# oceanusxiv/pathtracer-rs

Measured on NVIDIA B200. Metric: samples/sec, higher is better.
Workload: dtype f32

## Files before the change

pathtracer_rs_b200/csrc/dev_accel.cuh:

```cuda
#pragma once
#include "dev_texture.cuh"

namespace ptrs {

struct RayPre {
  int kz;
  float sx, sy, sz;
};
PT_DEV V3 permute(V3 v, int kz) {
  const bool z0 = kz == 0, z1 = kz == 1;
  return mk3(z0 ? v.y : (z1 ? v.z : v.x), z0 ? v.z : (z1 ? v.x : v.y), z0 ? v.x : (z1 ? v.y : v.z));
}

PT_DEV RayPre ray_precompute(V3 d) {
  RayPre p;
  p.kz = max_dimension(vabs(d));
  const V3 dp = permute(d, p.kz);
  p.sx = -dp.x / dp.z;
  p.sy = -dp.y / dp.z;
  p.sz = 1.0f / dp.z;
  return p;
}

PT_DEV bool tri_core(V3 p0, V3 p1, V3 p2, V3 o, const RayPre& rp, float t_max, float* t_out, float* b0o, float* b1o, float* b2o) {
// ... 203 lines not shown

#ifndef PT_REFILL_IDLE
#define PT_REFILL_IDLE 8
#endif
#ifndef PT_SEARCH_MIN
#define PT_SEARCH_MIN 6
#endif

template <class Work>
PT_DEV void trace_empty(uint32_t n_items, uint32_t* ticket, Work& work) {
  DevHit miss;
  miss.prim = -1;
  miss.t = miss.b0 = miss.b1 = miss.b2 = 0.f;
  const int lane = threadIdx.x & 31;
  for (;;) {
    const uint32_t base = (lane == 0) ? atomicAdd(ticket, 32u) : 0u;
    const uint32_t b = __shfl_sync(0xffffffffu, base, 0);
    if (b >= n_items) return;
    const uint32_t i = b + lane;
    if (i < n_items) {
      LaneRay r;
      bool more = work.begin(i, &r);
      while (more) more = work.end(i, miss, false, &r);
    }
  }
}

#define PT_RB_NX 1u
#define PT_RB_NY 2u
#define PT_RB_NZ 4u
#define PT_RB_KZ_SHIFT 3
#define PT_RB_ANY 32u
#define PT_RB_LIVE 64u
#ifndef PT_BOX_STEPS
#define PT_BOX_STEPS 3
#endif
#ifndef PT_TRI_STEPS
#define PT_TRI_STEPS 1
#endif
#ifndef PT_EAGER_POP
#define PT_EAGER_POP 0
#endif
#ifndef PT_NEAR_LEAF_DIRECT
#define PT_NEAR_LEAF_DIRECT 0
#endif
#ifndef PT_SMEM_STACK
#define PT_SMEM_STACK 0
#endif
#ifndef PT_STACK8
#define PT_STACK8 0
#endif
#ifndef PT_PUSH_PREFETCH
#define PT_PUSH_PREFETCH 0
#endif
#ifndef PT_PARK_PREFETCH_ON
#define PT_PARK_PREFETCH_ON 0
#endif
#if PT_PARK_PREFETCH_ON
#define PT_PARK_PREFETCH(prim) asm volatile("prefetch.global.L1 [%0];" ::"l"(sc.tri_verts + 3 * (size_t)(prim)))
#else
#define PT_PARK_PREFETCH(prim) ((void)0)
#endif

#ifndef PT_TRACE_BLOCK
#define PT_TRACE_BLOCK 128
#endif
// ... 674 lines not shown
        RayPre rp;
        rp.kz = (int)((rbits >> PT_RB_KZ_SHIFT) & 3u);
        rp.sx = sx;
        rp.sy = sy;
        rp.sz = sz;
        float t, b0, b1, b2;
        if (tri_core(mk3(v0), mk3(v1), mk3(v2), o, rp, t_max, &t, &b0, &b1, &b2) &&
            !tri_post_reject(sc, (int)prim, mk3(v0), mk3(v1), mk3(v2), __float_as_uint(v2.w), b0, b1, b2, false)) {
          hit_prim = (int)prim;
          pl_cnt = 0;
          sp_ = 0;
          cur = PT_W_NONE;
        }
      }
    };
    for (;;) {
      const bool has = pl_cnt != 0u || PT_W_IS_LEAF(cur);
      if (__ballot_sync(FULL, has) == 0) break;
      tri_step();
    }

    if ((rbits & PT_RB_LIVE) && cur == PT_W_NONE && sp_ == 0 && pl_cnt == 0u) {
      DevHit h;
      h.prim = hit_prim;
      h.t = t_max;
      h.b0 = h.b1 = h.b2 = 0.f;
      LaneRay r;
      if (work.end(item, h, hit_prim >= 0, &r)) start_ray(r);
      else rbits = 0;
    }
  }
}

template <bool COUNT, bool DIST, class Work>
PT_DEV void trace_stream(const DevScene& sc, uint32_t n_items, uint32_t* ticket, Work& work, uint32_t* c_nodes, uint32_t* c_tris) {
  if (COUNT) trace_counted(sc, n_items, ticket, work, c_nodes, c_tris);
  else trace_fast<DIST>(sc, n_items, ticket, work);
}

}
```

pathtracer_rs_b200/csrc/k_trace.cu:

```cuda
#include "launch.hpp"
#include "wavefront.cuh"

#ifndef PT_TRACE_MIN_BLOCKS
#define PT_TRACE_MIN_BLOCKS 8
#endif

namespace ptrs {

PT_DEV uint32_t coalesced_slot(uint32_t* counter) {
  const uint32_t m = __activemask();
  const uint32_t grp = __match_any_sync(m, (unsigned long long)(uintptr_t)counter);
  const int lane = threadIdx.x & 31;
  const int leader = __ffs(grp) - 1;
  uint32_t base = 0;
  if (lane == leader) base = atomicAdd(counter, (uint32_t)__popc(grp));
  base = __shfl_sync(grp, base, leader);
  return base + (uint32_t)__popc(grp & ((1u << lane) - 1u));
}

struct ExtendWork {
  const DevScene& sc;
  const PathArrays& P;
  const int* __restrict__ q_ext;
  int* __restrict__ q_class;
  uint32_t cap;
  RoundCounters* ctr;
  int p;
  __device__ bool begin(uint32_t i, LaneRay* r) {
    p = q_ext[i];
    const PathRay pr = ld256(&P.slot[p].r);
    r->o = mk3(pr.ox, pr.oy, pr.oz);
    r->d = mk3(pr.dx, pr.dy, pr.dz);
    r->t_max = CUDART_INF_F;
    r->any_hit = false;
    return true;
  }
  __device__ bool end(uint32_t, const DevHit& h, bool found, LaneRay*) {
    const int cls = found ? sc.materials[__float_as_int(__ldg(&sc.tri_verts[3 * (size_t)h.prim].w))].type : PT_CLASS_MISS;
    const size_t slot = (size_t)cls * cap + coalesced_slot(&ctr->n_class[cls]);
    q_class[slot] = p;
    if (found) P.q_hit[slot] = make_float4(__int_as_float(h.prim), h.b0, h.b1, h.b2);
    return false;
  }
};

template <bool COUNT, bool DIST>
__global__ void __launch_bounds__(128, PT_TRACE_MIN_BLOCKS) extend_kernel(const __grid_constant__ DevScene sc, const __grid_constant__ PathArrays P, const int* __restrict__ q_ext, int* __restrict__ q_class,
                                                      uint32_t cap, RoundCounters* ctr, GlobalCounters* g) {
  uint32_t c_nodes = 0, c_tris = 0;
  ExtendWork w{sc, P, q_ext, q_class, cap, ctr, 0};
  trace_stream<COUNT, DIST>(sc, ctr->n_ext, &ctr->t_ext, w, &c_nodes, &c_tris);
  if (COUNT) {
    warp_sum_add(c_nodes, &g->nodes_tested);
    warp_sum_add(c_tris, &g->tris_tested);
  }
}

struct ConnectWork {
  const PathArrays& P;
  uint32_t n_low, top;
  uint32_t n_shadow, n_mis;
  uint32_t cur;
  __device__ bool begin(uint32_t i, LaneRay* r) {
    cur = P.q_ray[i < n_low ? i : top - (i - n_low)];
    const uint32_t rec = cur >> 1;
    if (cur & 1u) {
      const F8 n23 = ld256(reinterpret_cast<const F8*>(&P.nee[rec].n2));
      r->o = mk3(n23.a);
      r->d = mk3(n23.b);
      r->t_max = CUDART_INF_F;
      r->any_hit = (__float_as_uint(n23.b.w) & PT_NEE_MIS_ANY) != 0;
      ++n_mis;
    } else {
      const F8 n01 = ld256(reinterpret_cast<const F8*>(&P.nee[rec].n0));
      r->o = mk3(n01.a);
      r->d = mk3(n01.b);
      r->t_max = 1.0f - PT_SHADOW_EPSILON;
      r->any_hit = true;
      ++n_shadow;
    }
    return true;
  }
  __device__ bool end(uint32_t, const DevHit& h, bool found, LaneRay*) {
    NeeRes* res = P.nee_res + (cur >> 1);
    if (cur & 1u) *reinterpret_cast<float4*>(res) = make_float4(__int_as_float(found ? h.prim : -1), h.b0, h.b1, h.b2);
    else res->occluded = found ? 1u : 0u;
    return false;
  }
};

template <bool COUNT, bool DIST>
__global__ void __launch_bounds__(128, PT_TRACE_MIN_BLOCKS) connect_kernel(const __grid_constant__ DevScene sc, const __grid_constant__ PathArrays P, uint32_t cap,
                                                                           bool closest_only, RoundCounters* ctr, GlobalCounters* g) {
  uint32_t c_nodes = 0, c_tris = 0;
  const uint32_t n_low = closest_only ? 0u : ctr->n_ray;
  ConnectWork w{P, n_low, 2u * cap - 1u, 0u, 0u, 0u};
  trace_stream<COUNT, DIST>(sc, n_low + ctr->n_ray_closest, closest_only ? &ctr->t_ray_closest : &ctr->t_ray, w, &c_nodes, &c_tris);
  warp_sum_add(w.n_shadow, &g->shadow_rays);
  warp_sum_add(w.n_mis, &g->mis_rays);
  if (COUNT) {
    warp_sum_add(c_nodes, &g->nee_nodes_tested);
    warp_sum_add(c_tris, &g->nee_tris_tested);
  }
}

__global__ void __launch_bounds__(128, PT_TRACE_MIN_BLOCKS) occlusion_kernel(const __grid_constant__ DevScene sc, const __grid_constant__ PathArrays P, RoundCounters* ctr, GlobalCounters* g) {
  const uint32_t n = ctr->n_ray;
  ConnectWork w{P, n, 0u, 0u, 0u, 0u};
  trace_occlusion(sc, n, &ctr->t_ray, w);
  warp_sum_add(w.n_shadow, &g->shadow_rays);
  warp_sum_add(w.n_mis, &g->mis_rays);
}

struct IntersectWork {
  const PtrsRay* __restrict__ rays;
  PtrsHit* __restrict__ hits;
  uint8_t* __restrict__ occluded;
  bool any_hit;
  const uint32_t* __restrict__ prim_map;
  __device__ bool begin(uint32_t i, LaneRay* r) {
    const float* q = (const float*)(rays + i);
    r->o = mk3(__ldg(q), __ldg(q + 1), __ldg(q + 2));
    r->d = mk3(__ldg(q + 3), __ldg(q + 4), __ldg(q + 5));
    r->t_max = __ldg(q + 6);
    r->any_hit = any_hit;
    return true;
  }
  __device__ bool end(uint32_t i, const DevHit& h, bool found, LaneRay*) {
    if (any_hit) {
      occluded[i] = found ? 1 : 0;
    } else {
      PtrsHit out;
      out.prim = found ? (prim_map ? (int)__ldg(prim_map + h.prim) : h.prim) : -1;
      out.t = found ? h.t : 0.f;
      out.b0 = h.b0;
      out.b1 = h.b1;
      out.b2 = h.b2;
      hits[i] = out;
    }
    return false;
  }
};

template <bool ANY_HIT, bool COUNT, bool DIST>
__global__ void __launch_bounds__(128, PT_TRACE_MIN_BLOCKS) intersect_kernel(const __grid_constant__ DevScene sc, const PtrsRay* __restrict__ rays, uint32_t n, PtrsHit* __restrict__ hits,
                                                         uint8_t* __restrict__ occluded, uint32_t* ticket, GlobalCounters* g, const uint32_t* __restrict__ prim_map) {
  uint32_t c_nodes = 0, c_tris = 0;
  IntersectWork w{rays, hits, occluded, ANY_HIT, prim_map};
  trace_stream<COUNT, DIST>(sc, n, ticket, w, &c_nodes, &c_tris);
  if (COUNT) {
    warp_sum_add(c_nodes, &g->nodes_tested);
    warp_sum_add(c_tris, &g->tris_tested);
  }
}

__global__ void __launch_bounds__(128, PT_TRACE_MIN_BLOCKS) intersect_p_occlusion_kernel(const __grid_constant__ DevScene sc, const PtrsRay* __restrict__ rays, uint32_t n,
                                                                                         uint8_t* __restrict__ occluded, uint32_t* ticket) {
  IntersectWork w{rays, nullptr, occluded, true, nullptr};
  trace_occlusion(sc, n, ticket, w);
}

void launch_extend(cudaStream_t st, int sm, bool count, const DevScene& sc, const PathArrays& P, const int* q_ext, int* q_class, uint32_t cap,
                   RoundCounters* ctr, GlobalCounters* g) {
  if (count) extend_kernel<true, false><<<PT_GRID((extend_kernel<true, false>), 128, sm), 128, 0, st>>>(sc, P, q_ext, q_class, cap, ctr, g);
  else if (sc.dist_order) extend_kernel<false, true><<<PT_GRID((extend_kernel<false, true>), 128, sm), 128, 0, st>>>(sc, P, q_ext, q_class, cap, ctr, g);
  else extend_kernel<false, false><<<PT_GRID((extend_kernel<false, false>), 128, sm), 128, 0, st>>>(sc, P, q_ext, q_class, cap, ctr, g);
}
void launch_connect(cudaStream_t st, int sm, bool count, const DevScene& sc, const PathArrays& P, uint32_t cap, bool closest_only, RoundCounters* ctr,
                    GlobalCounters* g) {
  if (count) connect_kernel<true, false><<<PT_GRID((connect_kernel<true, false>), 128, sm), 128, 0, st>>>(sc, P, cap, closest_only, ctr, g);
  else if (sc.dist_order) connect_kernel<false, true><<<PT_GRID((connect_kernel<false, true>), 128, sm), 128, 0, st>>>(sc, P, cap, closest_only, ctr, g);
  else connect_kernel<false, false><<<PT_GRID((connect_kernel<false, false>), 128, sm), 128, 0, st>>>(sc, P, cap, closest_only, ctr, g);
}
void launch_occlusion(cudaStream_t st, int sm, const DevScene& sc, const PathArrays& P, RoundCounters* ctr, GlobalCounters* g) {
  occlusion_kernel<<<PT_GRID(occlusion_kernel, 128, sm), 128, 0, st>>>(sc, P, ctr, g);
}
void launch_intersect(cudaStream_t st, int sm, bool any_hit, bool count, const DevScene& sc, const PtrsRay* rays, uint32_t n, PtrsHit* hits,
                      uint8_t* occluded, uint32_t* ticket, GlobalCounters* g, const uint32_t* prim_map) {
#define PT_LAUNCH_INTERSECT(A, C, D) \
  intersect_kernel<A, C, D><<<PT_GRID((intersect_kernel<A, C, D>), 128, sm), 128, 0, st>>>(sc, rays, n, hits, occluded, ticket, g, prim_map)
  const bool dist = sc.dist_order != 0;
  if (any_hit && !count && sc.n_wnodes > 0) intersect_p_occlusion_kernel<<<PT_GRID(intersect_p_occlusion_kernel, 128, sm), 128, 0, st>>>(sc, rays, n, occluded, ticket);
  else if (!any_hit && count) PT_LAUNCH_INTERSECT(false, true, false);
  else if (any_hit && count) PT_LAUNCH_INTERSECT(true, true, false);
  else if (!any_hit && dist) PT_LAUNCH_INTERSECT(false, false, true);
  else if (!any_hit) PT_LAUNCH_INTERSECT(false, false, false);
  else if (dist) PT_LAUNCH_INTERSECT(true, false, true);
  else PT_LAUNCH_INTERSECT(true, false, false);
#undef PT_LAUNCH_INTERSECT
}

}
```

pathtracer_rs_b200/csrc/ptrs_b200.cu:

```cuda
#include <cuda_runtime.h>

#include <algorithm>
#include <cmath>
#include <cstdio>
#include <cstdlib>
#include <cstring>
#include <memory>
#include <mutex>
#include <string>
#include <vector>

#include "handles.hpp"
#include "launch.hpp"
#include "wavefront.cuh"

using namespace ptrs;

extern "C" const unsigned char ptrs_sobol_blob[];
extern "C" const unsigned char ptrs_sobol_blob_end[];

namespace {

thread_local std::string g_err;
int32_t fail(int32_t code, const std::string& msg) {
  g_err = msg;
  return code;
}
}
int32_t ptrs::set_error(int32_t code, const std::string& msg) { return fail(code, msg); }
namespace {
#define CUDA_TRY(expr)                                                                                         \
  do {                                                                                                         \
    cudaError_t e__ = (expr);                                                                                  \
    if (e__ != cudaSuccess) return fail(PTRS_ERR_CUDA, std::string(#expr) + ": " + cudaGetErrorString(e__)); \
  } while (0)

struct SobolHost {
  uint32_t n_dims = 0, n_cols = 0;
  const uint32_t* matrices = nullptr;
  std::vector<std::vector<uint64_t>> vdc, vdc_inv;
  bool ok = false;
};
const SobolHost& sobol_host() {
  static SobolHost h;
// ... 426 lines not shown
        s->stats.launches += 1;
        s->stats.connect_launches += 1;
        s->stats.launches += 1;
      }
      tm.end();
      s->stats.launches += 1;
    }
    host_ctr.resize(round + 1);
    CUDA_TRY(cudaMemcpyAsync(host_ctr.data(), w.counters.p, (size_t)(round + 1) * sizeof(RoundCounters), cudaMemcpyDeviceToHost, st));
    CUDA_TRY(cudaStreamSynchronize(st));
    if (host_ctr[round].n_ext == 0 || round >= w.rounds) break;
  }
  for (uint32_t r = 0; r < round; ++r) *ext_rays += host_ctr[r].n_ext;
  if (host_ctr[round].n_ext != 0) return fail(PTRS_ERR_UNSUPPORTED, "paths still alive after the maximum number of wavefront rounds");
  return PTRS_OK;
}

}

extern "C" {

int32_t ptrs_abi_version(void) { return PTRS_ABI_VERSION; }
const char* ptrs_last_error(void) { return g_err.c_str(); }

int32_t ptrs_device_count(int32_t* count) {
  int n = 0;
  CUDA_TRY(cudaGetDeviceCount(&n));
  *count = n;
  return PTRS_OK;
}
int32_t ptrs_set_device(int32_t device) {
  CUDA_TRY(cudaSetDevice(device));
  return PTRS_OK;
}

static bool build_occlusion_tree(const PtrsBvhNode* nodes, uint32_t n_nodes, std::vector<float4>* out) {
  auto contains = [&](const PtrsBvhNode& a, const PtrsBvhNode& b) {
    for (int k = 0; k < 3; ++k)
      if (!(a.bounds_min[k] <= b.bounds_min[k]) || !(a.bounds_max[k] >= b.bounds_max[k])) return false;
    return true;
  };
  for (uint32_t i = 0; i < n_nodes; ++i) {
    const PtrsBvhNode& n = nodes[i];
    if (n.n_prims > 0) {
      if (n.n_prims > 16 || (uint64_t)n.offset + n.n_prims > (1u << 27)) return false;
    } else if (!contains(n, nodes[i + 1]) || !contains(n, nodes[n.offset])) {
      return false;
    }
  }
  auto area = [&](uint32_t i) {
    const PtrsBvhNode& n = nodes[i];
    const float dx = n.bounds_max[0] - n.bounds_min[0], dy = n.bounds_max[1] - n.bounds_min[1], dz = n.bounds_max[2] - n.bounds_min[2];
    return dx * dy + dy * dz + dz * dx;
  };
  out->clear();
  std::vector<std::pair<uint32_t, uint32_t>> todo{{0u, 0u}};
  out->resize(8);
  while (!todo.empty()) {
    const auto [r, w] = todo.back();
    todo.pop_back();
    std::vector<uint32_t> slot;
    if (nodes[r].n_prims > 0) slot.push_back(r);
    else slot = {r + 1, nodes[r].offset};
    while (slot.size() < 4) {
      int best = -1;
      for (int k = 0; k < (int)slot.size(); ++k)
        if (nodes[slot[k]].n_prims == 0 && (best < 0 || area(slot[k]) > area(slot[best]))) best = k;
      if (best < 0) break;
      const uint32_t c = slot[best];
      slot[best] = c + 1;
      slot.push_back(nodes[c].offset);
    }
    float lo[3][4], hi[3][4];
    uint32_t child[4];
    for (int k = 0; k < 4; ++k) {
      if (k >= (int)slot.size()) {
        for (int a = 0; a < 3; ++a) {
          lo[a][k] = INFINITY;
          hi[a][k] = -INFINITY;
        }
        child[k] = PT_W_NONE;
        continue;
      }
      const PtrsBvhNode& n = nodes[slot[k]];
      for (int a = 0; a < 3; ++a) {
        lo[a][k] = n.bounds_min[a];
        hi[a][k] = n.bounds_max[a];
      }
      if (n.n_prims > 0) {
        child[k] = PT_W_LEAF_BIT | ((uint32_t)(n.n_prims - 1) << 27) | n.offset;
      } else {
        child[k] = (uint32_t)(out->size() / 8);
        todo.emplace_back(slot[k], child[k]);
        out->resize(out->size() + 8);
      }
    }
    float4* rec = out->data() + 8 * (size_t)w;
    for (int a = 0; a < 3; ++a) {
      rec[2 * a] = make_float4(lo[a][0], lo[a][1], lo[a][2], lo[a][3]);
      rec[2 * a + 1] = make_float4(hi[a][0], hi[a][1], hi[a][2], hi[a][3]);
    }
    std::memcpy(&rec[6], child, 16);
    rec[7] = make_float4(0.f, 0.f, 0.f, 0.f);
  }
  return true;
}

static int32_t scene_create_impl(const PtrsSceneDesc* d, bool device_bvh, PtrsScene** out) {
  if (!d || !out) return fail(PTRS_ERR_INVALID_ARGUMENT, "null argument");
  if (d->abi_version != PTRS_ABI_VERSION) return fail(PTRS_ERR_INVALID_ARGUMENT, "PtrsSceneDesc.abi_version mismatch");
  if (d->n_prims > 0 && ((!device_bvh && !d->nodes) || !d->prim_vertex || !d->prim_mesh || !d->prim_material || !d->prim_area_light || !d->pos || !d->meshes))
    return fail(PTRS_ERR_INVALID_ARGUMENT, "missing geometry arrays");
  const SobolHost& sh = sobol_host();
  if (!sh.ok) return fail(PTRS_ERR_INVALID_ARGUMENT, "embedded Sobol tables are corrupt");
  int dev = 0;
  CUDA_TRY(cudaGetDevice(&dev));
  std::unique_ptr<PtrsScene> s(new PtrsScene());
  s->device = dev;
  CUDA_TRY(cudaDeviceGetAttribute(&s->sm_count, cudaDevAttrMultiProcessorCount, dev));
  uint32_t n_interior = 0;
  if (!device_bvh && d->n_prims > 0) {
    if (d->n_nodes == 0) return fail(PTRS_ERR_INVALID_ARGUMENT, "missing geometry arrays");
    std::vector<std::pair<uint32_t, uint32_t>> owed;
    bool prev_interior = false;
    uint32_t depth = 0, max_interior_depth = 0;
    for (uint32_t i = 0; i < d->n_nodes; ++i) {
      const PtrsBvhNode& n = d->nodes[i];
      if (i > 0 && !prev_interior) {
        if (owed.empty()) return fail(PTRS_ERR_INVALID_ARGUMENT, "malformed BVH (records after the end of the tree)");
        if (owed.back().first != i) return fail(PTRS_ERR_INVALID_ARGUMENT, "malformed BVH node (second child must follow the first child's subtree)");
        depth = owed.back().second;
        owed.pop_back();
      }
      if (n.n_prims > 0) {
        if ((uint64_t)n.offset + n.n_prims > d->n_prims) return fail(PTRS_ERR_INVALID_ARGUMENT, "malformed BVH node");
        prev_interior = false;
      } else {
        if (n.offset >= d->n_nodes || i + 1 >= d->n_nodes || n.axis > 2) return fail(PTRS_ERR_INVALID_ARGUMENT, "malformed BVH node");
// ... 92 lines not shown
      s->prim_map.p = perm;
      s->prim_map.n = d->n_prims;
      s->bvh_depth = dev_depth;
      if (dev_depth > PT_STACK_SIZE) return fail(PTRS_ERR_UNSUPPORTED, "device-built BVH deeper than the 64-entry traversal stack; build the tree on the host");
      launch_assemble_tris(0, d->n_prims, perm, pv.p, pos.p, pm.p, pmat.p, pal.p, s->meshes.p, s->tri_verts.p, s->tri_index.p, inv.p);
      launch_remap_light_prims(0, s->lights.p, d->n_lights, inv.p);
      CUDA_TRY(cudaEventRecord(e1, 0));
      CUDA_TRY(cudaEventSynchronize(e1));
      CUDA_TRY(cudaGetLastError());
      cudaEventElapsedTime(&s->bvh_build_ms, e0, e1);
      cudaEventDestroy(e0);
      cudaEventDestroy(e1);
      s->scene_bytes += (uint64_t)n_dev_nodes * 32 + (uint64_t)d->n_prims * 4;
      if (n_dev_nodes > 0) {
        float root[8];
        CUDA_TRY(cudaMemcpy(root, s->nodes.p, 32, cudaMemcpyDeviceToHost));
        s->world_bound[0] = root[0];
        s->world_bound[1] = root[1];
        s->world_bound[2] = root[2];
        s->world_bound[3] = root[3];
        s->world_bound[4] = root[4];
        s->world_bound[5] = root[5];
      }
    } else {
      static_assert(sizeof(PtrsBvhNode) == 32, "LinearBVHNode is 32 bytes");
      DevBuf<float4> raw;
      CUDA_TRY(raw.upload(reinterpret_cast<const float4*>(d->nodes), (size_t)d->n_nodes * 2));
      float4* nodes = nullptr;
      const int pe = pair_layout_on_device(0, raw.p, d->n_nodes, n_interior, &nodes, &n_dev_nodes);
      if (pe != (int)cudaSuccess) return fail(PTRS_ERR_CUDA, std::string("BVH re-layout: ") + cudaGetErrorString((cudaError_t)pe));
      s->nodes.p = nodes;
      s->nodes.n = (size_t)n_dev_nodes * 2;
      s->scene_bytes += (uint64_t)n_dev_nodes * 32;
      std::vector<float4> wide;
      if (build_occlusion_tree(d->nodes, d->n_nodes, &wide)) {
        CUDA_TRY(s->wnodes.upload(wide.data(), wide.size()));
        s->scene_bytes += (uint64_t)wide.size() * 16;
      }
      launch_assemble_tris(0, d->n_prims, nullptr, pv.p, pos.p, pm.p, pmat.p, pal.p, s->meshes.p, s->tri_verts.p, s->tri_index.p, nullptr);
      CUDA_TRY(cudaGetLastError());
      CUDA_TRY(cudaStreamSynchronize(0));
    }
  }
  if (n_dev_nodes > (1u << 30)) return fail(PTRS_ERR_UNSUPPORTED, "more than 2^30 BVH nodes");
  if (d->normal) CUDA_TRY(s->normal.upload(d->normal, (size_t)d->n_verts * 3));
  if (d->tangent) CUDA_TRY(s->tangent.upload(d->tangent, (size_t)d->n_verts * 3));
  if (d->uv) CUDA_TRY(s->uv.upload(d->uv, (size_t)d->n_verts * 2));
  CUDA_TRY(s->tri_shade.alloc((size_t)d->n_prims * 4));
  launch_pack_shading(0, d->n_prims, s->tri_verts.p, s->tri_index.p, s->normal.p, s->uv.p, s->tri_shade.p);
  CUDA_TRY(cudaGetLastError());
  CUDA_TRY(s->materials.upload(d->materials, d->n_materials));
  CUDA_TRY(s->textures.upload(d->textures, d->n_textures));
  {
    std::vector<PtrsMipMap> mips(d->mipmaps, d->mipmaps + d->n_mipmaps);
    std::vector<int> have(d->n_mipmaps, 0);
    bool build_any = false;
    uint64_t total = 0;
    for (uint32_t i = 0; i < d->n_mipmaps; ++i) {
      PtrsMipMap& m = mips[i];
      have[i] = m.n_levels;
      int want = 1;
      for (int e = std::max(m.width[0], m.height[0]); e > 1; e >>= 1) ++want;
      if (m.n_levels == 1 && want > 1) {
        if ((m.width[0] & (m.width[0] - 1)) || (m.height[0] & (m.height[0] - 1)))
          return fail(PTRS_ERR_UNSUPPORTED, "level 0 of a pyramid to be completed on the device must be a power of two in both axes (the Lanczos resample of MIPMap::new stays with the host)");
        if (want > PTRS_MAX_MIP_LEVELS) return fail(PTRS_ERR_INVALID_ARGUMENT, "MIP pyramid too deep");
        build_any = true;
        m.n_levels = want;
        for (int l = 1; l < want; ++l) {
          m.width[l] = std::max(1, m.width[l - 1] / 2);
// ... 739 lines not shown
```

pathtracer_rs_b200/host.py:

```python
import ctypes as C
import os

import numpy as np

from ._abi import *
from . import _abi

_HERE = os.path.dirname(os.path.abspath(__file__))
_LIB = None

SCENE_CORNELL, SCENE_CORNELL_ENV, SCENE_MATERIAL_FIELD, SCENE_TERRAIN, SCENE_ATRIUM = range(5)


def lib():
    global _LIB
    if _LIB is None:
        path = os.path.join(_HERE, "lib", "libptrs_host.so")
        if not os.path.exists(path):
            raise RuntimeError(f"{path} missing: run `python -c 'import __graft_entry__ as g; g.build()'`")
        L = C.CDLL(path)
        vp, i32, u32, u64, f32 = C.c_void_p, C.c_int, C.c_uint32, C.c_uint64, C.c_float
        fp = C.POINTER(C.c_float)
        L.ptrs_host_last_error.restype = C.c_char_p
        L.ptrs_host_builder_new.restype = vp
# ... 20 lines not shown
        L.ptrs_host_scene_desc_device_tables.argtypes = [vp]
        L.ptrs_host_scene_bytes_device_tables.restype = u64
        L.ptrs_host_scene_bytes_device_tables.argtypes = [vp]
        L.ptrs_host_scene_bvh_depth.argtypes = [vp]
        L.ptrs_host_scene_bvh_seconds.restype = C.c_double
        L.ptrs_host_scene_bvh_seconds.argtypes = [vp]
        L.ptrs_host_make_scene.restype = vp
        L.ptrs_host_make_scene.argtypes = [i32, u64, u64, i32, i32, C.POINTER(PtrsCamera), i32]
        L.ptrs_host_make_scene_env.restype = vp
        L.ptrs_host_make_scene_env.argtypes = [i32, u64, u64, i32, i32, C.POINTER(PtrsCamera), i32, C.c_char_p]
        L.ptrs_host_synth_sky.argtypes = [i32, i32, u64, fp]
        L.ptrs_host_make_camera.argtypes = [fp, fp, f32, f32, f32, f32, i32, i32, C.POINTER(PtrsCamera)]
        L.ptrs_host_mitsuba_camera.argtypes = [fp, f32, i32, i32, i32, i32, C.POINTER(PtrsCamera)]
        L.ptrs_host_look_at_camera.argtypes = [fp, fp, fp, f32, i32, i32, C.POINTER(PtrsCamera)]
        L.ptrs_host_default_render_params.argtypes = [C.POINTER(PtrsRenderParams)]
        L.ptrs_host_gaussian_filter_table.argtypes = [f32, f32, fp]
        L.ptrs_host_coherent_rays.argtypes = [C.POINTER(PtrsCamera), i32, C.POINTER(PtrsRay)]
        L.ptrs_host_incoherent_rays.argtypes = [fp, fp, u64, u64, C.POINTER(PtrsRay)]
        L.ptrs_host_import_scene.restype = vp
        L.ptrs_host_import_scene.argtypes = [C.c_char_p, i32, i32, i32, C.c_char_p, C.POINTER(PtrsCamera), i32]
        ip = C.POINTER(C.c_int)
        L.ptrs_host_load_hdr.argtypes = [C.c_char_p, ip, ip, fp]
        L.ptrs_host_save_hdr.argtypes = [C.c_char_p, fp, i32, i32]
        L.ptrs_host_load_png.argtypes = [C.c_char_p, ip, ip, ip, C.POINTER(C.c_uint8)]
        L.ptrs_host_save_png.argtypes = [C.c_char_p, C.POINTER(C.c_uint8), i32, i32, i32]
        L.ptrs_host_decode_image.argtypes = [C.POINTER(C.c_uint8), C.c_size_t, ip, ip, ip, C.POINTER(C.c_uint8)]
        L.ptrs_host_snake_case.argtypes = [C.c_char_p, C.c_char_p, i32]
        u8p = C.POINTER(C.c_uint8)
        L.ptrs_host_tev_create_image.restype = C.c_int64
        L.ptrs_host_tev_create_image.argtypes = [i32, i32, C.c_char_p, u8p, C.c_int64]
        L.ptrs_host_tev_update_image.restype = C.c_int64
        L.ptrs_host_tev_update_image.argtypes = [fp, i32, i32, C.c_char_p, u8p, C.c_int64]
        L.ptrs_host_build_bvh.argtypes = [fp, u32, i32, i32, C.POINTER(PtrsBvhNode), u32, C.POINTER(u32), C.POINTER(u32)]
        _LIB = L
    return _LIB


RAY_DTYPE = np.dtype([("o", np.float32, 3), ("d", np.float32, 3), ("t_max", np.float32)])
HIT_DTYPE = np.dtype([("prim", np.int32), ("t", np.float32), ("b0", np.float32), ("b1", np.float32), ("b2", np.float32)])
NODE_DTYPE = np.dtype([("bmin", np.float32, 3), ("bmax", np.float32, 3), ("offset", np.uint32),
                       ("n_prims", np.uint16), ("axis", np.uint8), ("pad", np.uint8)])
assert RAY_DTYPE.itemsize == 28 and HIT_DTYPE.itemsize == 20 and NODE_DTYPE.itemsize == 32


def _fp(a):
    return None if a is None else a.ctypes.data_as(C.POINTER(C.c_float))


def _f32(a, shape=None):
    if a is None:
        return None
    a = np.ascontiguousarray(a, dtype=np.float32)
    if shape is not None:
        a = a.reshape(shape)
    return a


class FlatScene:

    def __init__(self, handle):
        if not handle:
            raise RuntimeError("host scene build failed: " + lib().ptrs_host_last_error().decode(errors="replace"))
        self._h = handle
        self.desc = lib().ptrs_host_scene_desc(handle)

    def __del__(self):
        if getattr(self, "_h", None):
            try:
                lib().ptrs_host_scene_free(self._h)
            except TypeError:
                pass
            self._h = None

    @property
    def n_prims(self):
        return self.desc.contents.n_prims

    @property
    def n_nodes(self):
        return self.desc.contents.n_nodes

    @property
    def n_lights(self):
        return self.desc.contents.n_lights

    @property
    def host_bytes(self):
        return lib().ptrs_host_scene_bytes(self._h)

    @property
    def desc_device_tables(self):
        return lib().ptrs_host_scene_desc_device_tables(self._h)

    @property
    def host_bytes_device_tables(self):
        return lib().ptrs_host_scene_bytes_device_tables(self._h)

    @property
    def bvh_depth(self):
        return lib().ptrs_host_scene_bvh_depth(self._h)

    @property
    def bvh_seconds(self):
        return lib().ptrs_host_scene_bvh_seconds(self._h)

    def nodes(self):
        d = self.desc.contents
        return np.ctypeslib.as_array(C.cast(d.nodes, C.POINTER(C.c_uint8)), shape=(d.n_nodes * 32,)).view(NODE_DTYPE)

    def world_bound(self):
        n = self.nodes()[0]
        return np.array(n["bmin"]), np.array(n["bmax"])

    def prim_vertices(self):
        d = self.desc.contents
        idx = np.ctypeslib.as_array(d.prim_vertex, shape=(d.n_prims, 3))
        pos = np.ctypeslib.as_array(d.pos, shape=(d.n_verts, 3))
        return pos[idx]


TANK_FARM_HDR = os.path.join(os.path.dirname(_HERE), "tests", "golden", "abandoned_tank_farm_04_1k.hdr")


def make_scene(kind, seed=1, n_tris=0, res=(512, 512), n_threads=0, env_hdr=None):
    cam = PtrsCamera()
    h = lib().ptrs_host_make_scene_env(kind, seed, n_tris, res[0], res[1], C.byref(cam), n_threads, os.fsencode(env_hdr) if env_hdr else None)
    return FlatScene(h), cam


def import_scene(path, res=(640, 480), default_lights=False, sunsky_hdr=None, n_threads=0):
    cam = PtrsCamera()
    h = lib().ptrs_host_import_scene(os.fsencode(path), res[0], res[1], 1 if default_lights else 0,
                                     os.fsencode(sunsky_hdr) if sunsky_hdr else None, C.byref(cam), n_threads)
    return FlatScene(h), cam


def _img_check(rc):
    if rc != 0:
        raise RuntimeError(lib().ptrs_host_last_error().decode(errors="replace"))


# ... 193 lines not shown
```

pathtracer_rs_b200/host/capi.cpp:

```cpp
#include <cstring>
#include <exception>
#include <stdexcept>
#include <string>

#include "image_io.hpp"
#include "importers.hpp"
#include "procedural.hpp"
#include "scene_builder.hpp"
#include "tev.hpp"

using namespace ptrs_host;

namespace {
thread_local std::string g_err;
struct SceneBox {
  FlatScene fs;
  PtrsSceneDesc desc;
  PtrsSceneDesc slim;
};
template <class F>
int guard(F&& f) {
  try {
    f();
    return 0;
  } catch (const std::exception& e) {
    g_err = e.what();
    return -1;
  }
}
M4 to_m4(const float* m) {
  M4 r;
  if (m) std::memcpy(r.m, m, 64);
  else r = M4::identity();
  return r;
}
}

extern "C" {

const char* ptrs_host_last_error() { return g_err.c_str(); }

void* ptrs_host_builder_new() { return new SceneBuilder(); }
// ... 213 lines not shown
}
void ptrs_host_mitsuba_camera(const float* sensor16, float fov_deg, int film_w, int film_h, int res_w, int res_h,
                              PtrsCamera* out) {
  *out = mitsuba_camera(to_m4(sensor16), fov_deg, film_w, film_h, res_w, res_h);
}
void ptrs_host_look_at_camera(const float* eye, const float* target, const float* up, float fovy_deg, int w, int h,
                              PtrsCamera* out) {
  *out = look_at_camera(v3(eye[0], eye[1], eye[2]), v3(target[0], target[1], target[2]), v3(up[0], up[1], up[2]),
                        fovy_deg, w, h);
}
void ptrs_host_default_render_params(PtrsRenderParams* p) { default_render_params(p); }
void ptrs_host_gaussian_filter_table(float alpha, float radius, float* table256) {
  gaussian_filter_table(alpha, radius, table256);
}

void ptrs_host_coherent_rays(const PtrsCamera* cam, int side, PtrsRay* out) { coherent_rays(*cam, side, out); }
void ptrs_host_incoherent_rays(const float* mn, const float* mx, uint64_t seed, uint64_t n, PtrsRay* out) {
  incoherent_rays(mn, mx, seed, n, out);
}

int ptrs_host_build_bvh(const float* bounds6, uint32_t n, int max_prims, int n_threads, PtrsBvhNode* nodes_out,
                        uint32_t nodes_cap, uint32_t* n_nodes, uint32_t* prim_order_out) {
  return guard([&] {
    std::vector<Bounds3> b(n);
    std::memcpy(b.data(), bounds6, (size_t)n * 24);
    BvhBuildResult r = build_bvh(b, max_prims, n_threads);
    *n_nodes = (uint32_t)r.nodes.size();
    if (r.nodes.size() > nodes_cap) throw std::runtime_error("node capacity too small");
    std::memcpy(nodes_out, r.nodes.data(), r.nodes.size() * sizeof(PtrsBvhNode));
    std::memcpy(prim_order_out, r.prim_order.data(), (size_t)n * 4);
  });
}

}
```

Baseline: 228.9 million.

## Trace closest-hit rays through a 4-wide BVH with per-octant child ordering

Adds a closest-hit traversal over the 4-wide BVH, which until now served only occlusion. The wide-node builder moves to a shared host header and now stores a per-octant front-to-back child order. Extend, connect and closest-hit intersect kernels use this path whenever a wide tree exists, aiming to cut node visits and per-ray loads. A hit beyond t_max restarts the ray in an exact mode without distance culling, which adds complexity and extra work on those rays. Shadow and MIS ray counters move from begin() to end() so restarted rays are not counted twice.

```diff
diff --git a/pathtracer_rs_b200/csrc/dev_accel.cuh b/pathtracer_rs_b200/csrc/dev_accel.cuh
--- a/pathtracer_rs_b200/csrc/dev_accel.cuh
+++ b/pathtracer_rs_b200/csrc/dev_accel.cuh
@@ -259,6 +259,7 @@
 #define PT_RB_KZ_SHIFT 3
 #define PT_RB_ANY 32u
 #define PT_RB_LIVE 64u
+#define PT_RB_EXACT 128u
 #ifndef PT_BOX_STEPS
 #define PT_BOX_STEPS 3
 #endif
@@ -999,9 +1000,185 @@
   }
 }
 
-template <bool COUNT, bool DIST, class Work>
+template <class Work>
+PT_DEV void trace_wide(const DevScene& sc, uint32_t n_items, uint32_t* ticket, Work& work) {
+  const uint32_t FULL = 0xffffffffu;
+  const int box_min = (int)sc.box_min;
+  uint2 stack[PT_OSTACK_SIZE];
+  int sp_ = 0;
+  uint32_t cur = PT_W_NONE;
+  float cur_t = 0.f;
+  uint32_t pl_off = 0, pl_cnt = 0;
+  uint32_t rbits = 0;
+  bool exhausted = n_items == 0;
+  uint32_t item = 0;
+  V3 o = mk3(0, 0, 0), inv_dir = mk3(0, 0, 0);
+  float sx = 0.f, sy = 0.f, sz = 0.f;
+  float t_max = 0.f;
+  int hit_prim = -1;
+  float hit_b0 = 0.f, hit_b1 = 0.f, hit_b2 = 0.f;
+
+  auto start_ray = [&](const LaneRay& r) {
+    o = r.o;
+    inv_dir = mk3(1.0f / r.d.x, 1.0f / r.d.y, 1.0f / r.d.z);
+    const RayPre rp = ray_precompute(r.d);
+    sx = rp.sx;
+    sy = rp.sy;
+    sz = rp.sz;
+    rbits = PT_RB_LIVE | (inv_dir.x < 0.0f ? PT_RB_NX : 0u) | (inv_dir.y < 0.0f ? PT_RB_NY : 0u) | (inv_dir.z < 0.0f ? PT_RB_NZ : 0u) |
+            ((uint32_t)rp.kz << PT_RB_KZ_SHIFT) | (r.any_hit ? PT_RB_ANY : 0u);
+    t_max = r.t_max;
+    hit_prim = -1;
+    hit_b0 = hit_b1 = hit_b2 = 0.f;
+    sp_ = 0;
+    pl_cnt = 0;
+    cur = 0u;
+    cur_t = -CUDART_INF_F;
+  };
+  auto park = [&]() {
+    pl_off = PT_W_LEAF_OFF(cur);
+    pl_cnt = PT_W_LEAF_CNT(cur);
+    cur = PT_W_NONE;
+  };
+
+  for (;;) {
+    const uint32_t idle = __ballot_sync(FULL, !(rbits & PT_RB_LIVE));
+    if (!exhausted && (__popc(idle) >= PT_REFILL_IDLE)) {
+      const int lane = threadIdx.x & 31;
+      const int leader = __ffs(idle) - 1;
+      uint32_t base = 0;
+      if (lane == leader) base = atomicAdd(ticket, (uint32_t)__popc(idle));
+      base = __shfl_sync(FULL, base, leader);
+      if (base + (uint32_t)__popc(idle) >= n_items) exhausted = true;
+      if (!(rbits & PT_RB_LIVE)) {
+        const uint32_t i = base + (uint32_t)__popc(idle & ((1u << lane) - 1u));
+        if (i < n_items) {
+          LaneRay r;
+          if (work.begin(i, &r)) {
+            item = i;
+            start_ray(r);
+          }
+        }
+      }
+    }
+    if (__ballot_sync(FULL, rbits & PT_RB_LIVE) == 0) {
+      if (exhausted) break;
+      continue;
+    }
+
+    auto box_step = [&]() {
+      const bool exact = (rbits & PT_RB_EXACT) != 0u;
+      while (cur == PT_W_NONE && sp_ > 0) {
+        const uint2 e = stack[--sp_];
+        if (__uint_as_float(e.x) < ((exact && pl_cnt != 0u) ? CUDART_INF_F : t_max)) {
+          cur = e.y;
+          cur_t = __uint_as_float(e.x);
+        }
+      }
+      if (PT_W_IS_LEAF(cur) && pl_cnt == 0u) park();
+      if (!PT_W_IS_INTERIOR(cur)) return;
+      const float4* nd = sc.wnodes + 8 * (size_t)cur;
+      const float4 lx = __ldg(nd), hx = __ldg(nd + 1), ly = __ldg(nd + 2), hy = __ldg(nd + 3), lz = __ldg(nd + 4), hz = __ldg(nd + 5);
+      const uint4 ch = __ldg(reinterpret_cast<const uint4*>(nd + 6));
+      const uint2 ow = __ldg(reinterpret_cast<const uint2*>(nd + 7));
+      const bool nx = inv_dir.x < 0.0f, ny = inv_dir.y < 0.0f, nz = inv_dir.z < 0.0f;
+      const float cull = exact ? CUDART_INF_F : t_max;
+      auto geom = [&](float x0, float x1, float y0, float y1, float z0, float z1, uint32_t w, float* te) {
+        NodeLoad n;
+        n.a = make_float4(x0, y0, z0, x1);
+        n.b = make_float4(y1, z1, 0.f, 0.f);
+        return box_geom(n, o, inv_dir, nx, ny, nz, te) && *te < cull && w != PT_W_NONE;
+      };
+      float t0, t1, t2, t3;
+      const uint32_t acc = (geom(lx.x, hx.x, ly.x, hy.x, lz.x, hz.x, ch.x, &t0) ? 1u : 0u) | (geom(lx.y, hx.y, ly.y, hy.y, lz.y, hz.y, ch.y, &t1) ? 2u : 0u) |
+                           (geom(lx.z, hx.z, ly.z, hy.z, lz.z, hz.z, ch.z, &t2) ? 4u : 0u) | (geom(lx.w, hx.w, ly.w, hy.w, lz.w, hz.w, ch.w, &t3) ? 8u : 0u);
+      const uint32_t oct = rbits & 7u;
+      const uint32_t ord = ((oct & 4u) ? ow.y : ow.x) >> (8u * (oct & 3u));
+      cur = PT_W_NONE;
+#pragma unroll
+      for (int j = 3; j >= 0; --j) {
+        const uint32_t k = (ord >> (2 * j)) & 3u;
+        if ((acc >> k) & 1u) {
+          if (cur != PT_W_NONE && sp_ < PT_OSTACK_SIZE) stack[sp_++] = make_uint2(__float_as_uint(cur_t), cur);
+          cur = (k & 2u) ? ((k & 1u) ? ch.w : ch.z) : ((k & 1u) ? ch.y : ch.x);
+          cur_t = (k & 2u) ? ((k & 1u) ? t3 : t2) : ((k & 1u) ? t1 : t0);
+        }
+      }
+      if (exact && cur != PT_W_NONE && !(cur_t < (pl_cnt != 0u ? CUDART_INF_F : t_max))) cur = PT_W_NONE;
+      if (PT_W_IS_LEAF(cur) && pl_cnt == 0u) park();
+    };
+    for (;;) {
+      const bool live = (rbits & PT_RB_LIVE) != 0;
+      const bool can_box = PT_W_IS_INTERIOR(cur) || (cur == PT_W_NONE && sp_ > 0) || (PT_W_IS_LEAF(cur) && pl_cnt == 0u);
+      const uint32_t bmask = __ballot_sync(FULL, can_box);
+      if (bmask == 0) break;
+      if (__popc(bmask) < box_min && __ballot_sync(FULL, live && !can_box) != 0) break;
+#pragma unroll
+      for (int rep = 0; rep < PT_BOX_STEPS; ++rep) box_step();
+    }
+
+    auto tri_step = [&]() {
+      if (pl_cnt == 0u && PT_W_IS_LEAF(cur)) park();
+      if (pl_cnt != 0u) {
+        const uint32_t prim = pl_off;
+        const float4 v0 = __ldg(sc.tri_verts + 3 * (size_t)prim);
+        const float4 v1 = __ldg(sc.tri_verts + 3 * (size_t)prim + 1);
+        const float4 v2 = __ldg(sc.tri_verts + 3 * (size_t)prim + 2);
+        ++pl_off;
+        --pl_cnt;
+        RayPre rp;
+        rp.kz = (int)((rbits >> PT_RB_KZ_SHIFT) & 3u);
+        rp.sx = sx;
+        rp.sy = sy;
+        rp.sz = sz;
+        float t, b0, b1, b2;
+        if (tri_core(mk3(v0), mk3(v1), mk3(v2), o, rp, t_max, &t, &b0, &b1, &b2) &&
+            !tri_post_reject(sc, (int)prim, mk3(v0), mk3(v1), mk3(v2), __float_as_uint(v2.w), b0, b1, b2, !(rbits & PT_RB_ANY))) {
+          if (t > t_max && !(rbits & (PT_RB_EXACT | PT_RB_ANY))) {
+            LaneRay r;
+            work.begin(item, &r);
+            start_ray(r);
+            rbits |= PT_RB_EXACT;
+            return;
+          }
+          hit_prim = (int)prim;
+          hit_b0 = b0;
+          hit_b1 = b1;
+          hit_b2 = b2;
+          t_max = t;
+          if (rbits & PT_RB_ANY) {
+            pl_cnt = 0;
+            sp_ = 0;
+            cur = PT_W_NONE;
+          }
+        }
+        if (pl_cnt == 0u && cur != PT_W_NONE && !(cur_t < t_max)) cur = PT_W_NONE;
+      }
+    };
+    for (;;) {
+      const bool has = pl_cnt != 0u || PT_W_IS_LEAF(cur);
+      if (__ballot_sync(FULL, has) == 0) break;
+      tri_step();
+    }
+
+    if ((rbits & PT_RB_LIVE) && cur == PT_W_NONE && sp_ == 0 && pl_cnt == 0u) {
+      DevHit h;
+      h.prim = hit_prim;
+      h.t = t_max;
+      h.b0 = hit_b0;
+      h.b1 = hit_b1;
+      h.b2 = hit_b2;
+      LaneRay r;
+      if (work.end(item, h, hit_prim >= 0, &r)) start_ray(r);
+      else rbits = 0;
+    }
+  }
+}
+
+template <bool COUNT, bool DIST, bool WIDE, class Work>
 PT_DEV void trace_stream(const DevScene& sc, uint32_t n_items, uint32_t* ticket, Work& work, uint32_t* c_nodes, uint32_t* c_tris) {
   if (COUNT) trace_counted(sc, n_items, ticket, work, c_nodes, c_tris);
+  else if (WIDE) trace_wide(sc, n_items, ticket, work);
   else trace_fast<DIST>(sc, n_items, ticket, work);
 }
 
diff --git a/pathtracer_rs_b200/csrc/k_trace.cu b/pathtracer_rs_b200/csrc/k_trace.cu
--- a/pathtracer_rs_b200/csrc/k_trace.cu
+++ b/pathtracer_rs_b200/csrc/k_trace.cu
@@ -44,12 +44,12 @@
   }
 };
 
-template <bool COUNT, bool DIST>
+template <bool COUNT, bool DIST, bool WIDE>
 __global__ void __launch_bounds__(128, PT_TRACE_MIN_BLOCKS) extend_kernel(const __grid_constant__ DevScene sc, const __grid_constant__ PathArrays P, const int* __restrict__ q_ext, int* __restrict__ q_class,
                                                       uint32_t cap, RoundCounters* ctr, GlobalCounters* g) {
   uint32_t c_nodes = 0, c_tris = 0;
   ExtendWork w{sc, P, q_ext, q_class, cap, ctr, 0};
-  trace_stream<COUNT, DIST>(sc, ctr->n_ext, &ctr->t_ext, w, &c_nodes, &c_tris);
+  trace_stream<COUNT, DIST, WIDE>(sc, ctr->n_ext, &ctr->t_ext, w, &c_nodes, &c_tris);
   if (COUNT) {
     warp_sum_add(c_nodes, &g->nodes_tested);
     warp_sum_add(c_tris, &g->tris_tested);
@@ -70,18 +70,18 @@
       r->d = mk3(n23.b);
       r->t_max = CUDART_INF_F;
       r->any_hit = (__float_as_uint(n23.b.w) & PT_NEE_MIS_ANY) != 0;
-      ++n_mis;
     } else {
       const F8 n01 = ld256(reinterpret_cast<const F8*>(&P.nee[rec].n0));
       r->o = mk3(n01.a);
       r->d = mk3(n01.b);
       r->t_max = 1.0f - PT_SHADOW_EPSILON;
       r->any_hit = true;
-      ++n_shadow;
     }
     return true;
   }
   __device__ bool end(uint32_t, const DevHit& h, bool found, LaneRay*) {
+    if (cur & 1u) ++n_mis;
+    else ++n_shadow;
     NeeRes* res = P.nee_res + (cur >> 1);
     if (cur & 1u) *reinterpret_cast<float4*>(res) = make_float4(__int_as_float(found ? h.prim : -1), h.b0, h.b1, h.b2);
     else res->occluded = found ? 1u : 0u;
@@ -89,13 +89,13 @@
   }
 };
 
-template <bool COUNT, bool DIST>
+template <bool COUNT, bool DIST, bool WIDE>
 __global__ void __launch_bounds__(128, PT_TRACE_MIN_BLOCKS) connect_kernel(const __grid_constant__ DevScene sc, const __grid_constant__ PathArrays P, uint32_t cap,
                                                                            bool closest_only, RoundCounters* ctr, GlobalCounters* g) {
   uint32_t c_nodes = 0, c_tris = 0;
   const uint32_t n_low = closest_only ? 0u : ctr->n_ray;
   ConnectWork w{P, n_low, 2u * cap - 1u, 0u, 0u, 0u};
-  trace_stream<COUNT, DIST>(sc, n_low + ctr->n_ray_closest, closest_only ? &ctr->t_ray_closest : &ctr->t_ray, w, &c_nodes, &c_tris);
+  trace_stream<COUNT, DIST, WIDE>(sc, n_low + ctr->n_ray_closest, closest_only ? &ctr->t_ray_closest : &ctr->t_ray, w, &c_nodes, &c_tris);
   warp_sum_add(w.n_shadow, &g->shadow_rays);
   warp_sum_add(w.n_mis, &g->mis_rays);
   if (COUNT) {
@@ -142,12 +142,12 @@
   }
 };
 
-template <bool ANY_HIT, bool COUNT, bool DIST>
+template <bool ANY_HIT, bool COUNT, bool DIST, bool WIDE>
 __global__ void __launch_bounds__(128, PT_TRACE_MIN_BLOCKS) intersect_kernel(const __grid_constant__ DevScene sc, const PtrsRay* __restrict__ rays, uint32_t n, PtrsHit* __restrict__ hits,
                                                          uint8_t* __restrict__ occluded, uint32_t* ticket, GlobalCounters* g, const uint32_t* __restrict__ prim_map) {
   uint32_t c_nodes = 0, c_tris = 0;
   IntersectWork w{rays, hits, occluded, ANY_HIT, prim_map};
-  trace_stream<COUNT, DIST>(sc, n, ticket, w, &c_nodes, &c_tris);
+  trace_stream<COUNT, DIST, WIDE>(sc, n, ticket, w, &c_nodes, &c_tris);
   if (COUNT) {
     warp_sum_add(c_nodes, &g->nodes_tested);
     warp_sum_add(c_tris, &g->tris_tested);
@@ -160,34 +160,38 @@
   trace_occlusion(sc, n, ticket, w);
 }
 
+#define PT_LAUNCH_TRACE(K, ...) K<__VA_ARGS__><<<PT_GRID((K<__VA_ARGS__>), 128, sm), 128, 0, st>>>
 void launch_extend(cudaStream_t st, int sm, bool count, const DevScene& sc, const PathArrays& P, const int* q_ext, int* q_class, uint32_t cap,
                    RoundCounters* ctr, GlobalCounters* g) {
-  if (count) extend_kernel<true, false><<<PT_GRID((extend_kernel<true, false>), 128, sm), 128, 0, st>>>(sc, P, q_ext, q_class, cap, ctr, g);
-  else if (sc.dist_order) extend_kernel<false, true><<<PT_GRID((extend_kernel<false, true>), 128, sm), 128, 0, st>>>(sc, P, q_ext, q_class, cap, ctr, g);
-  else extend_kernel<false, false><<<PT_GRID((extend_kernel<false, false>), 128, sm), 128, 0, st>>>(sc, P, q_ext, q_class, cap, ctr, g);
+  if (count) PT_LAUNCH_TRACE(extend_kernel, true, false, false)(sc, P, q_ext, q_class, cap, ctr, g);
+  else if (sc.dist_order) PT_LAUNCH_TRACE(extend_kernel, false, true, false)(sc, P, q_ext, q_class, cap, ctr, g);
+  else if (sc.n_wnodes > 0) PT_LAUNCH_TRACE(extend_kernel, false, false, true)(sc, P, q_ext, q_class, cap, ctr, g);
+  else PT_LAUNCH_TRACE(extend_kernel, false, false, false)(sc, P, q_ext, q_class, cap, ctr, g);
 }
 void launch_connect(cudaStream_t st, int sm, bool count, const DevScene& sc, const PathArrays& P, uint32_t cap, bool closest_only, RoundCounters* ctr,
                     GlobalCounters* g) {
-  if (count) connect_kernel<true, false><<<PT_GRID((connect_kernel<true, false>), 128, sm), 128, 0, st>>>(sc, P, cap, closest_only, ctr, g);
-  else if (sc.dist_order) connect_kernel<false, true><<<PT_GRID((connect_kernel<false, true>), 128, sm), 128, 0, st>>>(sc, P, cap, closest_only, ctr, g);
-  else connect_kernel<false, false><<<PT_GRID((connect_kernel<false, false>), 128, sm), 128, 0, st>>>(sc, P, cap, closest_only, ctr, g);
+  if (count) PT_LAUNCH_TRACE(connect_kernel, true, false, false)(sc, P, cap, closest_only, ctr, g);
+  else if (sc.dist_order) PT_LAUNCH_TRACE(connect_kernel, false, true, false)(sc, P, cap, closest_only, ctr, g);
+  else if (sc.n_wnodes > 0) PT_LAUNCH_TRACE(connect_kernel, false, false, true)(sc, P, cap, closest_only, ctr, g);
+  else PT_LAUNCH_TRACE(connect_kernel, false, false, false)(sc, P, cap, closest_only, ctr, g);
 }
 void launch_occlusion(cudaStream_t st, int sm, const DevScene& sc, const PathArrays& P, RoundCounters* ctr, GlobalCounters* g) {
   occlusion_kernel<<<PT_GRID(occlusion_kernel, 128, sm), 128, 0, st>>>(sc, P, ctr, g);
 }
 void launch_intersect(cudaStream_t st, int sm, bool any_hit, bool count, const DevScene& sc, const PtrsRay* rays, uint32_t n, PtrsHit* hits,
                       uint8_t* occluded, uint32_t* ticket, GlobalCounters* g, const uint32_t* prim_map) {
-#define PT_LAUNCH_INTERSECT(A, C, D) \
-  intersect_kernel<A, C, D><<<PT_GRID((intersect_kernel<A, C, D>), 128, sm), 128, 0, st>>>(sc, rays, n, hits, occluded, ticket, g, prim_map)
+#define PT_LAUNCH_INTERSECT(A, C, D, W) PT_LAUNCH_TRACE(intersect_kernel, A, C, D, W)(sc, rays, n, hits, occluded, ticket, g, prim_map)
   const bool dist = sc.dist_order != 0;
   if (any_hit && !count && sc.n_wnodes > 0) intersect_p_occlusion_kernel<<<PT_GRID(intersect_p_occlusion_kernel, 128, sm), 128, 0, st>>>(sc, rays, n, occluded, ticket);
-  else if (!any_hit && count) PT_LAUNCH_INTERSECT(false, true, false);
-  else if (any_hit && count) PT_LAUNCH_INTERSECT(true, true, false);
-  else if (!any_hit && dist) PT_LAUNCH_INTERSECT(false, false, true);
-  else if (!any_hit) PT_LAUNCH_INTERSECT(false, false, false);
-  else if (dist) PT_LAUNCH_INTERSECT(true, false, true);
-  else PT_LAUNCH_INTERSECT(true, false, false);
+  else if (!any_hit && count) PT_LAUNCH_INTERSECT(false, true, false, false);
+  else if (any_hit && count) PT_LAUNCH_INTERSECT(true, true, false, false);
+  else if (!any_hit && dist) PT_LAUNCH_INTERSECT(false, false, true, false);
+  else if (!any_hit && sc.n_wnodes > 0) PT_LAUNCH_INTERSECT(false, false, false, true);
+  else if (!any_hit) PT_LAUNCH_INTERSECT(false, false, false, false);
+  else if (dist) PT_LAUNCH_INTERSECT(true, false, true, false);
+  else PT_LAUNCH_INTERSECT(true, false, false, false);
 #undef PT_LAUNCH_INTERSECT
 }
+#undef PT_LAUNCH_TRACE
 
 }
diff --git a/pathtracer_rs_b200/csrc/ptrs_b200.cu b/pathtracer_rs_b200/csrc/ptrs_b200.cu
--- a/pathtracer_rs_b200/csrc/ptrs_b200.cu
+++ b/pathtracer_rs_b200/csrc/ptrs_b200.cu
@@ -10,6 +10,7 @@
 #include <string>
 #include <vector>
 
+#include "../host/wide_tree.hpp"
 #include "handles.hpp"
 #include "launch.hpp"
 #include "wavefront.cuh"
@@ -502,78 +503,6 @@
 int32_t ptrs_set_device(int32_t device) {
   CUDA_TRY(cudaSetDevice(device));
   return PTRS_OK;
-}
-
-static bool build_occlusion_tree(const PtrsBvhNode* nodes, uint32_t n_nodes, std::vector<float4>* out) {
-  auto contains = [&](const PtrsBvhNode& a, const PtrsBvhNode& b) {
-    for (int k = 0; k < 3; ++k)
-      if (!(a.bounds_min[k] <= b.bounds_min[k]) || !(a.bounds_max[k] >= b.bounds_max[k])) return false;
-    return true;
-  };
-  for (uint32_t i = 0; i < n_nodes; ++i) {
-    const PtrsBvhNode& n = nodes[i];
-    if (n.n_prims > 0) {
-      if (n.n_prims > 16 || (uint64_t)n.offset + n.n_prims > (1u << 27)) return false;
-    } else if (!contains(n, nodes[i + 1]) || !contains(n, nodes[n.offset])) {
-      return false;
-    }
-  }
-  auto area = [&](uint32_t i) {
-    const PtrsBvhNode& n = nodes[i];
-    const float dx = n.bounds_max[0] - n.bounds_min[0], dy = n.bounds_max[1] - n.bounds_min[1], dz = n.bounds_max[2] - n.bounds_min[2];
-    return dx * dy + dy * dz + dz * dx;
-  };
-  out->clear();
-  std::vector<std::pair<uint32_t, uint32_t>> todo{{0u, 0u}};
-  out->resize(8);
-  while (!todo.empty()) {
-    const auto [r, w] = todo.back();
-    todo.pop_back();
-    std::vector<uint32_t> slot;
-    if (nodes[r].n_prims > 0) slot.push_back(r);
-    else slot = {r + 1, nodes[r].offset};
-    while (slot.size() < 4) {
-      int best = -1;
-      for (int k = 0; k < (int)slot.size(); ++k)
-        if (nodes[slot[k]].n_prims == 0 && (best < 0 || area(slot[k]) > area(slot[best]))) best = k;
-      if (best < 0) break;
-      const uint32_t c = slot[best];
-      slot[best] = c + 1;
-      slot.push_back(nodes[c].offset);
-    }
-    float lo[3][4], hi[3][4];
-    uint32_t child[4];
-    for (int k = 0; k < 4; ++k) {
-      if (k >= (int)slot.size()) {
-        for (int a = 0; a < 3; ++a) {
-          lo[a][k] = INFINITY;
-          hi[a][k] = -INFINITY;
-        }
-        child[k] = PT_W_NONE;
-        continue;
-      }
-      const PtrsBvhNode& n = nodes[slot[k]];
-      for (int a = 0; a < 3; ++a) {
-        lo[a][k] = n.bounds_min[a];
-        hi[a][k] = n.bounds_max[a];
-      }
-      if (n.n_prims > 0) {
-        child[k] = PT_W_LEAF_BIT | ((uint32_t)(n.n_prims - 1) << 27) | n.offset;
-      } else {
-        child[k] = (uint32_t)(out->size() / 8);
-        todo.emplace_back(slot[k], child[k]);
-        out->resize(out->size() + 8);
-      }
-    }
-    float4* rec = out->data() + 8 * (size_t)w;
-    for (int a = 0; a < 3; ++a) {
-      rec[2 * a] = make_float4(lo[a][0], lo[a][1], lo[a][2], lo[a][3]);
-      rec[2 * a + 1] = make_float4(hi[a][0], hi[a][1], hi[a][2], hi[a][3]);
-    }
-    std::memcpy(&rec[6], child, 16);
-    rec[7] = make_float4(0.f, 0.f, 0.f, 0.f);
-  }
-  return true;
 }
 
 static int32_t scene_create_impl(const PtrsSceneDesc* d, bool device_bvh, PtrsScene** out) {
@@ -732,10 +661,10 @@
       s->nodes.p = nodes;
       s->nodes.n = (size_t)n_dev_nodes * 2;
       s->scene_bytes += (uint64_t)n_dev_nodes * 32;
-      std::vector<float4> wide;
-      if (build_occlusion_tree(d->nodes, d->n_nodes, &wide)) {
-        CUDA_TRY(s->wnodes.upload(wide.data(), wide.size()));
-        s->scene_bytes += (uint64_t)wide.size() * 16;
+      std::vector<ptrs_host::WideNode> wide;
+      if (ptrs_host::build_wide_tree(d->nodes, d->n_nodes, &wide)) {
+        CUDA_TRY(s->wnodes.upload(reinterpret_cast<const float4*>(wide.data()), wide.size() * 8));
+        s->scene_bytes += (uint64_t)wide.size() * sizeof(ptrs_host::WideNode);
       }
       launch_assemble_tris(0, d->n_prims, nullptr, pv.p, pos.p, pm.p, pmat.p, pal.p, s->meshes.p, s->tri_verts.p, s->tri_index.p, nullptr);
       CUDA_TRY(cudaGetLastError());
diff --git a/pathtracer_rs_b200/host.py b/pathtracer_rs_b200/host.py
--- a/pathtracer_rs_b200/host.py
+++ b/pathtracer_rs_b200/host.py
@@ -76,6 +76,8 @@
         L.ptrs_host_tev_update_image.restype = C.c_int64
         L.ptrs_host_tev_update_image.argtypes = [fp, i32, i32, C.c_char_p, u8p, C.c_int64]
         L.ptrs_host_build_bvh.argtypes = [fp, u32, i32, i32, C.POINTER(PtrsBvhNode), u32, C.POINTER(u32), C.POINTER(u32)]
+        L.ptrs_host_wide_tree.restype = C.c_int64
+        L.ptrs_host_wide_tree.argtypes = [C.POINTER(PtrsBvhNode), u32, vp, u64]
         _LIB = L
     return _LIB
 
@@ -84,7 +86,8 @@
 HIT_DTYPE = np.dtype([("prim", np.int32), ("t", np.float32), ("b0", np.float32), ("b1", np.float32), ("b2", np.float32)])
 NODE_DTYPE = np.dtype([("bmin", np.float32, 3), ("bmax", np.float32, 3), ("offset", np.uint32),
                        ("n_prims", np.uint16), ("axis", np.uint8), ("pad", np.uint8)])
-assert RAY_DTYPE.itemsize == 28 and HIT_DTYPE.itemsize == 20 and NODE_DTYPE.itemsize == 32
+WIDE_NODE_DTYPE = np.dtype([("planes", np.float32, (3, 2, 4)), ("child", np.uint32, 4), ("order", np.uint8, 8), ("pad", np.uint32, 2)])
+assert RAY_DTYPE.itemsize == 28 and HIT_DTYPE.itemsize == 20 and NODE_DTYPE.itemsize == 32 and WIDE_NODE_DTYPE.itemsize == 128
 
 
 def _fp(a):
@@ -151,6 +154,14 @@
     def nodes(self):
         d = self.desc.contents
         return np.ctypeslib.as_array(C.cast(d.nodes, C.POINTER(C.c_uint8)), shape=(d.n_nodes * 32,)).view(NODE_DTYPE)
+
+    def wide_tree(self):
+        d = self.desc.contents
+        n = lib().ptrs_host_wide_tree(d.nodes, d.n_nodes, None, 0)
+        out = np.zeros(n, dtype=WIDE_NODE_DTYPE)
+        if n:
+            lib().ptrs_host_wide_tree(d.nodes, d.n_nodes, out.ctypes.data_as(C.c_void_p), n)
+        return out
 
     def world_bound(self):
         n = self.nodes()[0]
diff --git a/pathtracer_rs_b200/host/capi.cpp b/pathtracer_rs_b200/host/capi.cpp
--- a/pathtracer_rs_b200/host/capi.cpp
+++ b/pathtracer_rs_b200/host/capi.cpp
@@ -8,6 +8,7 @@
 #include "procedural.hpp"
 #include "scene_builder.hpp"
 #include "tev.hpp"
+#include "wide_tree.hpp"
 
 using namespace ptrs_host;
 
@@ -287,4 +288,11 @@
   });
 }
 
-}
+int64_t ptrs_host_wide_tree(const PtrsBvhNode* nodes, uint32_t n_nodes, void* out, uint64_t cap) {
+  std::vector<WideNode> wide;
+  if (!build_wide_tree(nodes, n_nodes, &wide)) return 0;
+  if (wide.size() <= cap) std::memcpy(out, wide.data(), wide.size() * sizeof(WideNode));
+  return (int64_t)wide.size();
+}
+
+}
diff --git a/pathtracer_rs_b200/host/wide_tree.hpp b/pathtracer_rs_b200/host/wide_tree.hpp
--- /dev/null
+++ b/pathtracer_rs_b200/host/wide_tree.hpp
@@ -0,0 +1,111 @@
+#pragma once
+#include <cmath>
+#include <cstdint>
+#include <utility>
+#include <vector>
+
+#include "../../include/ptrs_b200.h"
+
+namespace ptrs_host {
+
+constexpr uint32_t kWideNone = 0xffffffffu;
+constexpr uint32_t kWideLeafBit = 0x80000000u;
+
+struct WideNode {
+  float lo_x[4], hi_x[4], lo_y[4], hi_y[4], lo_z[4], hi_z[4];
+  uint32_t child[4];
+  uint8_t order[8];
+  uint32_t pad[2];
+};
+static_assert(sizeof(WideNode) == 128, "wide node records are 128 bytes");
+
+inline bool build_wide_tree(const PtrsBvhNode* nodes, uint32_t n_nodes, std::vector<WideNode>* out) {
+  out->clear();
+  if (n_nodes == 0) return false;
+  auto contains = [&](const PtrsBvhNode& a, const PtrsBvhNode& b) {
+    for (int k = 0; k < 3; ++k)
+      if (!(a.bounds_min[k] <= b.bounds_min[k]) || !(a.bounds_max[k] >= b.bounds_max[k])) return false;
+    return true;
+  };
+  for (uint32_t i = 0; i < n_nodes; ++i) {
+    const PtrsBvhNode& n = nodes[i];
+    if (n.n_prims > 0) {
+      if (n.n_prims > 16 || (uint64_t)n.offset + n.n_prims > (1u << 27)) return false;
+    } else if (!contains(n, nodes[i + 1]) || !contains(n, nodes[n.offset])) {
+      return false;
+    }
+  }
+  auto area = [&](uint32_t i) {
+    const PtrsBvhNode& n = nodes[i];
+    const float dx = n.bounds_max[0] - n.bounds_min[0], dy = n.bounds_max[1] - n.bounds_min[1], dz = n.bounds_max[2] - n.bounds_min[2];
+    return dx * dy + dy * dz + dz * dx;
+  };
+  std::vector<std::pair<uint32_t, uint32_t>> todo{{0u, 0u}};
+  out->resize(1);
+  while (!todo.empty()) {
+    const auto [r, w] = todo.back();
+    todo.pop_back();
+    std::vector<uint32_t> slot;
+    if (nodes[r].n_prims > 0) slot.push_back(r);
+    else slot = {r + 1, nodes[r].offset};
+    while (slot.size() < 4) {
+      int best = -1;
+      for (int k = 0; k < (int)slot.size(); ++k)
+        if (nodes[slot[k]].n_prims == 0 && (best < 0 || area(slot[k]) > area(slot[best]))) best = k;
+      if (best < 0) break;
+      const uint32_t c = slot[best];
+      slot[best] = c + 1;
+      slot.push_back(nodes[c].offset);
+    }
+    WideNode rec{};
+    for (int k = 0; k < 4; ++k) {
+      float lo[3] = {INFINITY, INFINITY, INFINITY}, hi[3] = {-INFINITY, -INFINITY, -INFINITY};
+      rec.child[k] = kWideNone;
+      if (k < (int)slot.size()) {
+        const PtrsBvhNode& n = nodes[slot[k]];
+        for (int a = 0; a < 3; ++a) {
+          lo[a] = n.bounds_min[a];
+          hi[a] = n.bounds_max[a];
+        }
+        if (n.n_prims > 0) {
+          rec.child[k] = kWideLeafBit | ((uint32_t)(n.n_prims - 1) << 27) | n.offset;
+        } else {
+          rec.child[k] = (uint32_t)out->size();
+          todo.emplace_back(slot[k], rec.child[k]);
+          out->emplace_back();
+        }
+      }
+      rec.lo_x[k] = lo[0];
+      rec.hi_x[k] = hi[0];
+      rec.lo_y[k] = lo[1];
+      rec.hi_y[k] = hi[1];
+      rec.lo_z[k] = lo[2];
+      rec.hi_z[k] = hi[2];
+    }
+    for (int oct = 0; oct < 8; ++oct) {
+      uint32_t ord = 0, pos = 0, used = 0;
+      std::vector<uint32_t> walk{r};
+      while (!walk.empty()) {
+        const uint32_t x = walk.back();
+        walk.pop_back();
+        int k = 0;
+        while (k < (int)slot.size() && slot[k] != x) ++k;
+        if (k < (int)slot.size()) {
+          ord |= (uint32_t)k << (2 * pos++);
+          used |= 1u << k;
+          continue;
+        }
+        const bool neg = (oct >> nodes[x].axis) & 1;
+        walk.push_back(neg ? x + 1 : nodes[x].offset);
+        walk.push_back(neg ? nodes[x].offset : x + 1);
+      }
+      for (uint32_t k = 0; k < 4; ++k)
+        if (!(used & (1u << k))) ord |= k << (2 * pos++);
+      rec.order[oct] = (uint8_t)ord;
+    }
+    (*out)[w] = rec;
+  }
+  return true;
+}
+
+}
```

New measurement: 225.3 million (median of 6 runs). 0.985x the previous value.
